# polimi-ispl/deep_prior_interpolation

Hardware: AMD Instinct MI355X
Metric: Adam iters/sec on 3D MultiRes-UNet (whole job over n_gpus; per_gpu beside it); recon SNR(dB) vs ref under config.snr_vs_reference (higher is better)
Workload: dtype f32

## Files before the change

### deep_prior_interpolation_amd/_lib.py

```python
import ctypes as C
import os

_HERE = os.path.dirname(os.path.abspath(__file__))
LIB_PATH = os.path.join(_HERE, "libdpi_hip.so")


class DpiError(RuntimeError):
    pass


ABI_VERSION = 406

IO_X_BF16, IO_Y_BF16, IO_DY_BF16, IO_DX_BF16 = 1, 2, 4, 8
STORE_FWD_BF16, STORE_GRAD_BF16 = 1, 2


class ConvDesc(C.Structure):
    _fields_ = [("size", C.c_int), ("Cin", C.c_int), ("Cout", C.c_int), ("D", C.c_int), ("H", C.c_int), ("W", C.c_int),
                ("k", C.c_int), ("kd", C.c_int), ("stride", C.c_int), ("precision", C.c_int), ("io", C.c_int)]

    def __init__(self, Cin=0, Cout=0, D=1, H=1, W=1, k=1, kd=1, stride=1, precision=0, io=0):
        super().__init__(C.sizeof(ConvDesc), int(Cin), int(Cout), int(D), int(H), int(W), int(k), int(kd), int(stride), int(precision), int(io))


# ... 11 lines not shown

SIGNATURES = {
    "dpi_last_error": (C.c_char_p, []),
    "dpi_version": (_I, []),
    "dpi_conv_desc_size": (_I, []),
    "dpi_device_info": (_I, [_I, C.POINTER(_I), C.POINTER(_I), C.POINTER(_Z), C.c_char_p, _I]),
    "dpi_profile_marker": (_I, [_I, _P]),
    "dpi_conv_fwd_stat_blocks": (_I, [_DESC]),
    "dpi_conv_fwd": (_I, [_DESC, _P, _P, _P, _P, _P, _P, _P]),
    "dpi_conv_bwd_data": (_I, [_DESC, _P, _P, _P, _I, _P]),
    "dpi_conv_fwd_ws_floats": (_Z, [_DESC]),
    "dpi_conv_bwd_data_ws_floats": (_Z, [_DESC]),
    "dpi_conv_fwd_ws": (_I, [_DESC, _P, _P, _P, _P, _P, _P, _P, _Z, _P]),
    "dpi_conv_bwd_data_ws": (_I, [_DESC, _P, _P, _P, _I, _P, _Z, _P]),
    "dpi_conv_bwd_data_dual": (_I, [_DESC, _P, _P, _DESC, _P, _P, _P, _I, _P, _Z, _P]),
    "dpi_conv_bwd_weight_ws_floats": (_Z, [_DESC]),
    "dpi_conv_bwd_weight": (_I, [_DESC, _P, _P, _P, _P, _P, _Z, _P]),
    "dpi_stat_blocks": (_I, [_I, _Z]),
    "dpi_channel_stats": (_I, [_P, _P, _I, _Z, _P, _P]),
    "dpi_bn_finalize": (_I, [_P, _I, _I, _Z, _P, _P, _F, _F, _F, _I, _P, _P, _P, _P, _P, _P, _P]),
    "dpi_chain_apply": (_I, [_P, _P, _I, _Z, _P, _P]),
    "dpi_bn_bwd_reduce": (_I, [_P, _P, _P, _P, _P, _P, _F, _F, _I, _Z, _P, _P]),
    "dpi_bn_bwd_apply": (_I, [_P, _P, _P, _P, _P, _P, _F, _F, _P, _I, _I, _Z, _P, _P, _P, _P]),
    "dpi_bn_bwd_apply_fork": (_I, [_P, _P, _P, _P, _P, _P, _F, _F, _P, _I, _I, _Z, _P, _P, _P,
                                   _P, _P, _P, _P, _P, _F, _P, _P, _P, _P, _P, _P, _F, _P, _P]),
    "dpi_bn_bwd_apply_dual": (_I, [_P, _I, _I, _Z] + [_P, _P, _P, _P, _P, _F, _P, _P, _P, _P] * 2 + [_I, _I, _P, _P, _P, _F, _P, _P]),
    "dpi_chain_add_stats": (_I, [_P, _P, _P, _P, _I, _Z, _F, _P, _P, _P]),
    "dpi_lrelu_bwd": (_I, [_P, _P, _F, _Z, _P, _P]),
    "dpi_act_fwd": (_I, [_P, _Z, _I, _P, _P]),
    "dpi_act_bwd": (_I, [_P, _P, _Z, _I, _P, _P]),
# ... 99 lines not shown
```

### deep_prior_interpolation_amd/csrc/api.cpp

```cpp
#include <stdarg.h>
#include <string.h>
#include "common.h"

static thread_local char g_err[512] = "";

void dpi_set_error(const char* fmt, ...) {
  va_list ap;
  va_start(ap, fmt);
  vsnprintf(g_err, sizeof(g_err), fmt, ap);
  va_end(ap);
}

int dpi_check_launch(const char* what) {
  const hipError_t e = hipGetLastError();
  if (e != hipSuccess) {
    dpi_set_error("%s: %s", what, hipGetErrorString(e));
    return DPI_E_LAUNCH;
  }
  return DPI_OK;
}

extern "C" const char* dpi_last_error(void) { return g_err; }
extern "C" int dpi_version(void) { return 406; }
extern "C" int dpi_conv_desc_size(void) { return (int)sizeof(dpi_conv_desc); }
// ... 17 lines not shown

__global__ void dpi_marker_kernel() {}

extern "C" int dpi_profile_marker(int id, void* stream) {
  DPI_REQUIRE(id >= 1 && id < 65536, "profile_marker: id %d out of range", id);
  dpi_marker_kernel<<<(unsigned)id, 64, 0, (hipStream_t)stream>>>();
  return dpi_check_launch("profile_marker");
}

extern "C" int dpi_set_option(const char* key, int value) {
  DPI_REQUIRE(key != nullptr, "set_option: key is NULL");
  struct Entry { const char* key; int lo, hi; void (*set)(int); };
  static const Entry table[] = {
      {"splitk", 0, 1, dpi_set_splitk},
      {"dual_bwd_data", 0, 1, dpi_set_dual_bwd_data},
      {"bw_pair", 0, 2, dpi_set_bw_pair},
      {"bw_workgroups", 1, 1 << 24, [](int v) { dpi_set_bw_tuning(v, -1); }},
      {"bw_xcd_order", 0, 1, [](int v) { dpi_set_bw_tuning(0, v); }},
      {"mfma_min_cout", 0, 1 << 20, dpi_set_mfma_min_cout},
      {"bwd_weight_mfma_min_cout", 0, 1 << 20, dpi_set_bwd_weight_mfma_min_cout},
      {"fewco_mfma", 0, 1, dpi_set_fewco_mfma},
      {"q4", 0, 2, [](int v) { dpi_set_q4(v, -1); }},
      {"q4_ck", 0, 4, [](int v) { dpi_set_q4(-1, v); }},
      {"q4_debug", 0, 0xFFFF, dpi_set_q4_debug},
      {"bf16_debug", 0, 0x7F, dpi_set_bf16_debug},
  };
  for (const Entry& e : table)
    if (strcmp(key, e.key) == 0) {
      DPI_REQUIRE(value >= e.lo && value <= e.hi && !(strcmp(key, "q4_ck") == 0 && value != 0 && value != 2 && value != 4),
                  "set_option: %s = %d out of range [%d, %d]", key, value, e.lo, e.hi);
// ... 7 lines not shown
```

### deep_prior_interpolation_amd/csrc/conv_direct.hip

```cpp
#include "conv_kernels.h"

namespace {

struct ConvArgs {
  const float* __restrict__ x;
  const float* __restrict__ chain;
  const float* __restrict__ w;
  const float* __restrict__ bias;
  float* __restrict__ y;
  double* __restrict__ partials;
  int Cin, Cout;
  int D, H, W;
  int Do, Ho, Wo;
  int ntd, nth, ntw;
  long w_out_stride, w_in_stride;
  int accumulate;
  int xb, yb;
};

template <int KD, int S, int CO_B, int OW, int TZ, int TY, int TX, int CI_B, bool FLIP>
__global__ __launch_bounds__(TZ* TY* TX) void conv_direct_kernel(ConvArgs a) {
  constexpr int KS = 3;
  constexpr int NT = TZ * TY * TX;
  constexpr int SD = (KD > 1) ? S : 1;
// ... 485 lines not shown
}

extern "C" int dpi_conv_fwd_ws(const dpi_conv_desc* d, const float* x, const float* x_chain, const float* w, const float* bias, float* y,
                               double* stat_partials, float* ws, size_t ws_floats, void* stream) {
  if (int e = dpi_check_conv_desc(d)) return e;
  DPI_REQUIRE(x && w && y, "conv_fwd: null tensor");
  DPI_REQUIRE(ws || ws_floats == 0, "conv_fwd: workspace size without a workspace");
  return conv_run(d, x, x_chain, w, bias, y, stat_partials, false, 0, ws, ws_floats, (hipStream_t)stream);
}

extern "C" int dpi_conv_fwd(const dpi_conv_desc* d, const float* x, const float* x_chain, const float* w,
                            const float* bias, float* y, double* stat_partials, void* stream) {
  return dpi_conv_fwd_ws(d, x, x_chain, w, bias, y, stat_partials, nullptr, 0, stream);
}

extern "C" int dpi_conv_bwd_data(const dpi_conv_desc* d, const float* dy, const float* w, float* dx,
                                 int accumulate, void* stream) {
  return dpi_conv_bwd_data_ws(d, dy, w, dx, accumulate, nullptr, 0, stream);
}

static int g_dual = getenv("DPI_NO_DUAL") ? 0 : 1;
extern "C" void dpi_set_dual_bwd_data(int on) { g_dual = on; }
extern "C" int dpi_conv_bwd_data_dual(const dpi_conv_desc* d3, const float* dy3, const float* w3, const dpi_conv_desc* d1, const float* dy1,
                                      const float* w1, float* dx, int accumulate, float* ws, size_t ws_floats, void* stream) {
  if (int e = dpi_check_conv_desc(d3)) return e;
  if (int e = dpi_check_conv_desc(d1)) return e;
  DPI_REQUIRE(dy3 && w3 && dy1 && w1 && dx, "conv_bwd_data_dual: null tensor");
  DPI_REQUIRE(ws || ws_floats == 0, "conv_bwd_data_dual: workspace size without a workspace");
  DPI_REQUIRE(d3->k == 3 && d1->k == 1 && d3->stride == 1 && d1->stride == 1, "conv_bwd_data_dual: needs a 3x3(x3) and a 1x1(x1) stride-1 layer");
  DPI_REQUIRE(d3->Cin == d1->Cin && d3->D == d1->D && d3->H == d1->H && d3->W == d1->W, "conv_bwd_data_dual: the two layers read different tensors");
// ... 33 lines not shown
```

### deep_prior_interpolation_amd/csrc/conv_kernels.h

```cpp
#pragma once
#include "common.h"

struct MfmaSecond { const float* x2; const float* w2; int C2; long w2_co_stride, w2_c_stride; };
void dpi_conv_out_dims(const dpi_conv_desc* d, int* Do, int* Ho, int* Wo);
int dpi_conv_mfma_stat_blocks(const dpi_conv_desc* d, bool flip);
size_t dpi_conv_mfma_ws_floats(const dpi_conv_desc* d, bool flip);
bool dpi_conv_mfma_second_ok(const dpi_conv_desc* d, bool flip, int C2, bool have_ws);
int dpi_conv_mfma_run(const dpi_conv_desc* d, const float* x, const float* chain, const float* w, const float* bias, float* y,
                      double* partials, bool flip, int accumulate, float* ws, size_t ws_floats, hipStream_t st, const MfmaSecond* sec = nullptr);
int dpi_conv_bwd_data_s2_mfma_run(const dpi_conv_desc* d, const float* dy, const float* w, float* dx, int accumulate, hipStream_t st);
size_t dpi_conv_bwd_weight_mfma_ws_floats(const dpi_conv_desc* d);
bool dpi_conv_bwd_weight_mfma_swapped(const dpi_conv_desc* d, bool chained);
int dpi_conv_bwd_weight_mfma_run(const dpi_conv_desc* d, const float* x, const float* chain, const float* dy, float* dw, float* ws, hipStream_t st);
size_t dpi_conv_bwd_weight_smallco_ws_floats(const dpi_conv_desc* d);
int dpi_conv_bwd_weight_smallco_run(const dpi_conv_desc* d, const float* x, const float* chain, const float* dy, float* dw, float* ws, hipStream_t st);
int dpi_conv_pw_mfma_stat_blocks(const dpi_conv_desc* d);
int dpi_conv_pw_mfma_run(const dpi_conv_desc* d, const float* x, const float* chain, const float* w, const float* bias, float* y,
                         double* partials, bool flip, int accumulate, hipStream_t st);
size_t dpi_conv_pw_bwd_weight_mfma_ws_floats(const dpi_conv_desc* d);
int dpi_conv_pw_bwd_weight_mfma_run(const dpi_conv_desc* d, const float* x, const float* chain, const float* dy, float* dw, float* ws, hipStream_t st);
bool dpi_conv_fewco_usable(const dpi_conv_desc* d);
int dpi_conv_fewco_stat_blocks(const dpi_conv_desc* d);
int dpi_conv_fewco_mfma_run(const dpi_conv_desc* d, const float* x, const float* chain, const float* w, const float* bias, float* y,
                            double* partials, hipStream_t st);
bool dpi_conv_q4_usable(const dpi_conv_desc* d, bool flip);
int dpi_conv_q4_stat_blocks(const dpi_conv_desc* d);
int dpi_conv_q4_run(const dpi_conv_desc* d, const float* x, const float* chain, const float* w, const float* bias, float* y,
                    double* partials, bool flip, int accumulate, hipStream_t st);
bool dpi_bf16_force_all();
bool dpi_conv_bf16_usable(const dpi_conv_desc* d, bool flip);
int dpi_conv_bf16_stat_blocks(const dpi_conv_desc* d);
bool dpi_conv_bf16_second_ok(const dpi_conv_desc* d, bool flip);
int dpi_conv_bf16_run(const dpi_conv_desc* d, const float* x, const float* chain, const float* w, const float* bias, float* y,
                      double* partials, bool flip, int accumulate, hipStream_t st, const MfmaSecond* sec = nullptr);
bool dpi_conv_bf16_s2_usable(const dpi_conv_desc* d);
int dpi_conv_bf16_s2_stat_blocks(const dpi_conv_desc* d);
int dpi_conv_bf16_s2_run(const dpi_conv_desc* d, const float* x, const float* chain, const float* w, const float* bias, float* y, double* partials,
                         hipStream_t st);
bool dpi_conv_bf16_s2_bwd_usable(const dpi_conv_desc* d);
int dpi_conv_bf16_s2_bwd_run(const dpi_conv_desc* d, const float* dy, const float* w, float* dx, int accumulate, hipStream_t st);
bool dpi_conv_bf16_bww_usable(const dpi_conv_desc* d);
size_t dpi_conv_bf16_bww_ws_floats(const dpi_conv_desc* d);
int dpi_conv_bf16_bww_run(const dpi_conv_desc* d, const float* x, const float* chain, const float* dy, float* dw, float* ws, hipStream_t st);
// ... 4 lines not shown
```

### deep_prior_interpolation_amd/csrc/conv_q4_mfma.hip

```cpp
#include "conv_kernels.h"

namespace {

typedef float f32x4 __attribute__((ext_vector_type(4)));

struct QArgs {
  const float* __restrict__ x;
  const float* __restrict__ chain;
  const float* __restrict__ w;
  const float* __restrict__ bias;
  float* __restrict__ y;
  double* __restrict__ partials;
  int Cin, Cout;
  int D, H, W;
  int ntd, nth, ntw;
  long w_out_stride, w_in_stride;
  int accumulate;
  int dbg;
};

template <int R>
struct QGeo {
  static constexpr int TZ = 4, TY = R, TW = 64;
  static constexpr int ID = TZ + 2, IH = R + 2;
  static constexpr int RS = 72;
  static constexpr int DS = IH * RS, CS = ID * DS;
  static constexpr int NV4 = ID * IH * 18;
  static constexpr int E = (NV4 + 255) / 256;
};

__device__ __forceinline__ int q4_xcd_tile(int bid, int ntiles) {
  const int q = ntiles >> 3, r = ntiles & 7, xcd = bid & 7, i = bid >> 3;
  return (xcd < r ? xcd * (q + 1) : r * (q + 1) + (xcd - r) * q) + i;
// ... 202 lines not shown

template <int R>
struct QiGeo {
  static constexpr int TZ = 4, TY = R, TW = 64;
  static constexpr int ID = TZ + 2, IH = R + 2;
  static constexpr int NP = 72;
  static constexpr int RS = NP * 4, DS = IH * RS, TILE = ID * DS;
  static constexpr int NSLOT = ID * IH * 18;
  static constexpr int E = (NSLOT + 255) / 256;
};
__device__ __forceinline__ int qi_pos(int col) {
  const int g = col >> 2, j = col & 3;
  return (4 * g + (j ^ ((g >> 1) & 3))) * 4;
}

template <int R, int NB, bool FLIP, bool AL, bool KHP = false>
__global__ __launch_bounds__(256, 2) void conv_q4i_mfma_kernel(QArgs a) {
  static_assert(!KHP || (NB == 1 && !FLIP), "kh-packed rows: one output channel, forward only");
  using G = QiGeo<R>;
  constexpr int TAPS = 27;
  constexpr int NWT = KHP ? 9 * 16 : TAPS * NB * 16;
  constexpr int WE = (NWT + 255) / 256;
  __shared__ __attribute__((aligned(16))) float lds[G::TILE];
  __shared__ __attribute__((aligned(16))) float wl[NWT];
  __shared__ double red[4][4 * NB][2];

  const int tid = threadIdx.x, lane = tid & 63, wid = tid >> 6;
  const int ntiles = a.ntd * a.nth * a.ntw;
  const int tile_id = q4_xcd_tile(blockIdx.x, ntiles);
  int bt = tile_id;
  const int tw_i = bt % a.ntw; bt /= a.ntw;
  const int th_i = bt % a.nth; bt /= a.nth;
  const int od0 = bt * G::TZ, oh0 = th_i * G::TY, ow0 = tw_i * G::TW;
  const size_t V = (size_t)a.D * a.H * a.W;

  int goff[G::E], loff[G::E];
#pragma unroll
  for (int e = 0; e < G::E; ++e) {
    const int idx = tid + e * 256;
    const int q = idx % 18, row = idx / 18;
    const int hy = row % G::IH, dz = row / G::IH;
    const int gd = od0 - 1 + dz, gh = oh0 - 1 + hy, gw = ow0 - 4 + 4 * q;
    const bool ok = idx < G::NSLOT && gd >= 0 && gd < a.D && gh >= 0 && gh < a.H && gw >= 0 && gw + 4 <= a.W;
    goff[e] = ok ? (gd * a.H + gh) * a.W + gw : -4;
    loff[e] = idx < G::NSLOT ? dz * G::DS + hy * G::RS + 16 * q : -1;
  }
  const int swz = ((tid % 18) >> 1) & 3;
  auto stage_load = [&](f32x4 (&sr)[G::E][4], int c0) {
#pragma unroll
    for (int c = 0; c < 4; ++c) {
      const int ci = min(c0 + c, a.Cin - 1);
      const __amdgpu_buffer_rsrc_t r = dpi_buffer(a.x + (size_t)ci * V, V * sizeof(float));
#pragma unroll
      for (int e = 0; e < G::E; ++e) {
        if constexpr (AL) sr[e][c] = __builtin_bit_cast(f32x4, __builtin_amdgcn_raw_buffer_load_b128(r, goff[e] * 4, 0, 0));
        else {
#pragma unroll
          for (int k = 0; k < 4; ++k) sr[e][c][k] = dpi_buffer_load(r, goff[e] < 0 ? -4 : (goff[e] + k) * 4);
        }
// ... 44 lines not shown
  auto load_wt = [&](float (&wreg)[WE], int c0) {
#pragma unroll
    for (int k = 0; k < WE; ++k) {
      bool ok;
      wreg[k] = a.w[wt_index(tid + k * 256, c0, ok)];
    }
  };
  auto store_wt = [&](const float (&wreg)[WE], int c0) {
#pragma unroll
    for (int k = 0; k < WE; ++k) {
      bool ok;
      wt_index(tid + k * 256, c0, ok);
      if (tid + k * 256 < NWT) wl[tid + k * 256] = ok ? wreg[k] : 0.f;
    }
  };

  const int Do = a.D, Ho = a.H, Wo = a.W;
  const int od = od0 + wid, ow = ow0 + lane;
  f32x4 acc[R][NB];
#pragma unroll
  for (int hr = 0; hr < R; ++hr)
#pragma unroll
    for (int s = 0; s < NB; ++s) acc[hr][s] = (f32x4){0.f, 0.f, 0.f, 0.f};
  f32x4 accp[KHP ? G::IH : 1][2];
#pragma unroll
  for (int q = 0; q < (KHP ? G::IH : 1); ++q) { accp[q][0] = (f32x4){0.f, 0.f, 0.f, 0.f}; accp[q][1] = (f32x4){0.f, 0.f, 0.f, 0.f}; }

  f32x4 sr[G::E][4];
  float wreg[WE];
  load_wt(wreg, 0);
  stage_load(sr, 0);

  int xoff[3];
#pragma unroll
  for (int kw = 0; kw < 3; ++kw) xoff[kw] = wid * G::DS + qi_pos(3 + lane + kw);
  const f32x4* __restrict__ wl4 = reinterpret_cast<const f32x4*>(wl) + (lane & 3);

  for (int c0 = 0; c0 < a.Cin; c0 += 4) {
    __syncthreads();
    if (!(a.dbg & 2) || c0 == 0) stage_store(sr, c0);
    store_wt(wreg, c0);
    __syncthreads();
    auto load_x = [&](f32x4 (&xv)[3], int kd, int ir) {
#pragma unroll
      for (int kw = 0; kw < 3; ++kw) xv[kw] = *reinterpret_cast<const f32x4*>(lds + xoff[kw] + kd * G::DS + ir * G::RS);
    };
    auto load_w = [&](f32x4 (&wr)[9][NB], int kd) {
      if constexpr (KHP) {
#pragma unroll
        for (int kw = 0; kw < 3; ++kw) wr[kw][0] = wl4[(kd * 3 + kw) * 4];
      } else {
#pragma unroll
        for (int t = 0; t < 9; ++t)
#pragma unroll
          for (int s = 0; s < NB; ++s) wr[t][s] = wl4[((kd * 9 + t) * NB + s) * 4];
      }
    };
    f32x4 wr[9][NB], xv[3], xn[3];
    load_w(wr, 0);
    load_x(xv, 0, 0);
    __builtin_amdgcn_sched_barrier(0);
    if (c0 + 4 < a.Cin) {
      load_wt(wreg, c0 + 4);
      if (!(a.dbg & 1)) stage_load(sr, c0 + 4);
    }
    __builtin_amdgcn_sched_barrier(0);
#pragma unroll
    for (int kd = 0; kd < 3; ++kd) {
#pragma unroll
      for (int ir = 0; ir < G::IH; ++ir) {
        if (ir + 1 < G::IH) load_x(xn, kd, ir + 1);
        else if (kd + 1 < 3) load_x(xn, kd + 1, 0);
        __builtin_amdgcn_sched_barrier(0);
        if constexpr (KHP) {
#pragma unroll
          for (int kw = 0; kw < 3; ++kw)
#pragma unroll
            for (int c = 0; c < 4; ++c)
              accp[ir][c & 1] = __builtin_amdgcn_mfma_f32_4x4x1f32(wr[kw][0][c], xv[kw][c], accp[ir][c & 1], 0, 0, 0);
        } else {
#pragma unroll
        for (int kw = 0; kw < 3; ++kw)
#pragma unroll
          for (int c = 0; c < 4; ++c)
#pragma unroll
            for (int kh = 0; kh < 3; ++kh) {
              const int hr = ir - kh;
              if (hr >= 0 && hr < R) {
#pragma unroll
                for (int s = 0; s < NB; ++s)
                  acc[hr][s] = __builtin_amdgcn_mfma_f32_4x4x1f32(wr[kh * 3 + kw][s][c], xv[kw][c], acc[hr][s], 0, 0, 0);
              }
            }
        }
        __builtin_amdgcn_sched_barrier(0);
#pragma unroll
        for (int kw = 0; kw < 3; ++kw) xv[kw] = xn[kw];
      }
      if (kd + 1 < 3) load_w(wr, kd + 1);
    }
  }

  if constexpr (KHP) {
#pragma unroll
    for (int hr = 0; hr < R; ++hr)
      acc[hr][0][0] = ((accp[hr][0][0] + accp[hr][1][0]) + (accp[hr + 1][0][1] + accp[hr + 1][1][1])) + (accp[hr + 2][0][2] + accp[hr + 2][1][2]);
  }
  const bool col_ok = od < Do && ow < Wo;
#pragma unroll
  for (int s = 0; s < NB; ++s)
#pragma unroll
    for (int i = 0; i < 4; ++i) {
      const int co = 4 * s + i;
      const bool cok = co < a.Cout;
      const float bv = (a.bias && cok) ? a.bias[co] : 0.f;
      float* __restrict__ yc = a.y + (size_t)(cok ? co : 0) * V + ((size_t)(od < Do ? od : 0) * Ho + oh0) * Wo + ow;
      double sm = 0.0, sq = 0.0;
      float old[R];
      if (a.accumulate) {
#pragma unroll
        for (int hr = 0; hr < R; ++hr) old[hr] = (cok && col_ok && oh0 + hr < Ho) ? yc[hr * Wo] : 0.f;
      } else {
#pragma unroll
        for (int hr = 0; hr < R; ++hr) old[hr] = 0.f;
      }
#pragma unroll
      for (int hr = 0; hr < R; ++hr) {
        if (cok && col_ok && oh0 + hr < Ho) {
          const float v = acc[hr][s][i] + bv + old[hr];
          if (!(a.dbg & 8)) yc[hr * Wo] = v;
          sm += v;
          sq += (double)v * v;
        }
      }
      if (a.partials && cok) {
        sm = wave_sum(sm);
        sq = wave_sum(sq);
        if (lane == 0) { red[wid][co][0] = sm; red[wid][co][1] = sq; }
      }
    }
  if (a.partials) {
    __syncthreads();
    if (tid < 2 * a.Cout) {
      const int c = tid >> 1, which = tid & 1;
      a.partials[((size_t)tile_id * a.Cout + c) * 2 + which] = red[0][c][which] + red[1][c][which] + red[2][c][which] + red[3][c][which];
    }
  }
}

static int g_q4 = 1;
static int g_q4_ck = 0;
static int g_q4_dbg = 0;
static int g_q4_khp = getenv("DPI_NO_KHP") ? 0 : 1;

}

extern "C" void dpi_set_q4_debug(int flags) { g_q4_dbg = flags; }
extern "C" void dpi_set_q4(int on, int ck) {
  if (on >= 0) g_q4 = on;
  if (ck == 0 || ck == 2 || ck == 4) g_q4_ck = ck;
// ... 36 lines not shown
  if (aligned) conv_q4_mfma_kernel<8, NB, 2, FLIP, true><<<ntiles, 256, extra, st>>>(a);
  else conv_q4_mfma_kernel<8, NB, 2, FLIP, false><<<ntiles, 256, extra, st>>>(a);
}

int dpi_conv_q4_run(const dpi_conv_desc* d, const float* x, const float* chain, const float* w, const float* bias, float* y,
                    double* partials, bool flip, int accumulate, hipStream_t st) {
  const int cin = flip ? d->Cout : d->Cin, cout = flip ? d->Cin : d->Cout;
  const long w_out = flip ? 27 : (long)d->Cin * 27, w_in = flip ? (long)d->Cin * 27 : 27;
  QArgs a{x, chain, w, bias, y, partials, cin, cout, d->D, d->H, d->W, 0, 0, 0, w_out, w_in, accumulate, g_q4_dbg};
  const int ntiles = q4_tiles(d, &a.ntd, &a.nth, &a.ntw);
  const bool aligned = ((uintptr_t)x & 15) == 0;
  if (cout <= 4) { if (flip) q4_launch<1, true>(a, ntiles, aligned, st); else q4_launch<1, false>(a, ntiles, aligned, st); }
  else { if (flip) q4_launch<2, true>(a, ntiles, aligned, st); else q4_launch<2, false>(a, ntiles, aligned, st); }
  return dpi_check_launch("conv_q4_mfma");
}
```

### deep_prior_interpolation_amd/csrc/dpi_hip_internal.h

```cpp
#pragma once
#define DPI_INTERNAL __attribute__((visibility("hidden")))
extern "C" {
DPI_INTERNAL void dpi_set_bw_tuning(int want_workgroups, int xcd_order);
DPI_INTERNAL void dpi_set_bf16_debug(int flags);
DPI_INTERNAL void dpi_set_splitk(int on);
DPI_INTERNAL void dpi_set_dual_bwd_data(int on);
DPI_INTERNAL void dpi_set_bw_pair(int mode);
DPI_INTERNAL void dpi_set_mfma_min_cout(int n);
DPI_INTERNAL void dpi_set_bwd_weight_mfma_min_cout(int n);
DPI_INTERNAL void dpi_set_fewco_mfma(int on);
DPI_INTERNAL void dpi_set_q4(int on, int ck);
DPI_INTERNAL void dpi_set_q4_debug(int flags);
}
```

### deep_prior_interpolation_amd/ops.py

```python
import ctypes as C
import os
import threading

import torch

from . import _lib
from ._lib import ConvDesc, check, ptr, stream

BN_EPS = 1e-5
BN_MOMENTUM = 0.1


def _req(t, name, act=False):
    if not t.is_cuda:
        raise _lib.DpiError("%s must live on the GPU: the HIP path has no CPU fallback" % name)
    if t.dtype != torch.float32 and not (act and t.dtype == torch.bfloat16):
        raise _lib.DpiError("%s must be float32%s (got %s)" % (name, " or bfloat16" if act else "", t.dtype))
    return t.contiguous()


STORAGE_BF16 = os.environ.get("DPI_STORAGE", "fp32") == "bf16"
_tls = threading.local()


# ... 162 lines not shown
_ws_cache = {}


def _ws_floats(kind, d):
    key = (kind, d.Cin, d.Cout, d.D, d.H, d.W, d.k, d.kd, d.stride, d.precision, d.io)
    n = _ws_cache.get(key)
    if n is None:
        L = _lib.load()
        n = {"fwd": L.dpi_conv_fwd_ws_floats, "bwd_data": L.dpi_conv_bwd_data_ws_floats}[kind](C.byref(d))
        _ws_cache[key] = n
    return n


def reset_ws_cache():
    _ws_cache.clear()


def _conv_ws(n, like):
    return torch.empty(n, dtype=torch.float32, device=like.device) if n else None


def raw_conv_fwd(d, x, chain, w, bias, y, partials=None):
    L = _lib.load()
    n = _ws_floats("fwd", d)
    ws = _conv_ws(n, x)
    _timed("conv_fwd", d, lambda: check(L.dpi_conv_fwd_ws(C.byref(d), ptr(x), ptr(chain), ptr(w), ptr(bias), ptr(y),
                                                          ptr(partials), ptr(ws), n, stream()), "dpi_conv_fwd"))


def raw_conv_bwd_data(d, dy, w, dx, accumulate=False):
    L = _lib.load()
    n = _ws_floats("bwd_data", d)
    ws = _conv_ws(n, dy)
    _timed("conv_bwd_data", d, lambda: check(L.dpi_conv_bwd_data_ws(C.byref(d), ptr(dy), ptr(w), ptr(dx), int(accumulate),
                                                                    ptr(ws), n, stream()), "dpi_conv_bwd_data"))


def raw_conv_bwd_data_dual(d3, dy3, w3, d1, dy1, w1, dx, accumulate=False):
    L = _lib.load()
    n = _ws_floats("bwd_data", d3)
    ws = _conv_ws(n, dy3)

# ... 471 lines not shown
                raw_conv_bwd_data(d, dr, w, dx)
        if ctx.has_bias and ctx.needs_input_grad[2]:
            db = _zeros_like_or_none(ctx.bias_ref, dr)
        join_weight_grads()
        return dx, dw, db, dgamma, dbeta, None, None, None, None, None, None


def _cba_raw(d, x, in_chain, w, b, bn, slope, r_out, mi_out, chain_out):
    L = _lib.load()
    nblk = L.dpi_conv_fwd_stat_blocks(C.byref(d))
    part = torch.empty(nblk * d.Cout * 2, dtype=torch.float64, device=x.device)
    raw_conv_fwd(d, x, in_chain, w, b, r_out, part)
    Do, Ho, Wo = desc_out_dims(d)
    raw_bn_finalize(part, nblk, d.Cout, Do * Ho * Wo, bn.weight, bn.bias, slope, bn.running_mean, bn.running_var,
                    bn.num_batches_tracked, mi_out, chain_out)


DEAD_BIAS = "off"


def _zeros_like_or_none(b, dr=None):
    if b is None or DEAD_BIAS == "off":
        return None
    if DEAD_BIAS == "noise":
        return torch.randn_like(b) * 1e-6
    return dr.sum(dim=[0] + list(range(2, dr.ndim)), dtype=torch.float32)


class Block3dFn(torch.autograd.Function):

# ... 16 lines not shown
        r1, r2, r3 = R[:, :c1], R[:, c1:c1 + c2], R[:, c1 + c2:]
        ch1, ch2, ch3 = CH[:c1 * 5], CH[c1 * 5:(c1 + c2) * 5], CH[(c1 + c2) * 5:]
        mi1, mi2, mi3 = (torch.empty(2 * c, **f32) for c in (c1, c2, c3))
        miA, miS, miB = (torch.empty(2 * Ct, **f32) for _ in range(3))
        dsc = make_desc(x, ws, 1, adt)
        S = torch.empty_like(R)
        chSA = torch.empty((2, Ct * 5), **f32)
        chS, chA = chSA[0], chSA[1]
        side_shortcut = BRANCH_SHORTCUT if branch_on() else 0

        def shortcut_on_branch():
            with _Branch("short", x, S, miS, chS):
                _cba_raw(dsc, x, None, ws, bs, bns_, slope, S, miS, chS)
        if side_shortcut == 1:
            shortcut_on_branch()
        _cba_raw(d1, x, None, w1, b1, bn1_, slope, r1, mi1, ch1)
        if side_shortcut == 2:
            shortcut_on_branch()
        d2 = make_desc(r1, w2, 1, adt)
        _cba_raw(d2, r1, ch1, w2, b2, bn2_, slope, r2, mi2, ch2)
        d3 = make_desc(r2, w3, 1, adt)
        _cba_raw(d3, r2, ch2, w3, b3, bn3_, slope, r3, mi3, ch3)
        A = blk.bn1
        raw_bn_stats_finalize(R, CH, Ct, V, gA, eA, 1.0, A.running_mean, A.running_var, A.num_batches_tracked, miA, chA,
                              compose=True)
        if side_shortcut:
            join_branch("short")
        else:
            _cba_raw(dsc, x, None, ws, bs, bns_, slope, S, miS, chS)
        y = torch.empty_like(R)
        tless = _join_fused_ok(R, S)
        t = _join_forward(S, chS, R, chA, Ct, V, slope, blk.bn2, gB, eB, miB, y, keep_t=not tless)
        if tless:
            t = chSA
        ctx.tless = tless
        ctx.save_for_backward(x, R, S, t, CH, mi1, mi2, mi3, miA, miS, miB, *[q for q in p if q is not None])
        ctx.none_mask = [q is None for q in p]
        ctx.descs = (d1, d2, d3, dsc)
        ctx.slope = float(slope)
        ctx.split = (c1, c2, c3)
        return y

    @staticmethod
# ... 63 lines not shown
        x = _req(x, "respath input", act=True)
        (w3, b3, g3, e3, w1, b1, g1, e1, gB, eB) = p
        L = _lib.load()
        f32 = dict(dtype=torch.float32, device=x.device)
        adt = act_dtype()
        Ct = w3.shape[0]
        bn3_, bn1_ = rp.conv3x3._parts()[1], rp.conv1x1._parts()[1]
        d3, d1 = make_desc(x, w3, 1, adt), make_desc(x, w1, 1, adt)
        Do, Ho, Wo = desc_out_dims(d3)
        V = Do * Ho * Wo
        r3 = torch.empty(_like_spatial(x, Ct, Do, Ho, Wo), dtype=adt, device=x.device)
        r1 = torch.empty_like(r3)
        mi3, mi1, miB = (torch.empty(2 * Ct, **f32) for _ in range(3))
        ch13 = torch.empty((2, 5 * Ct), **f32)
        ch1, ch3 = ch13[0], ch13[1]
        _cba_raw(d3, x, None, w3, b3, bn3_, slope, r3, mi3, ch3)
        _cba_raw(d1, x, None, w1, b1, bn1_, slope, r1, mi1, ch1)
        y = torch.empty_like(r3)
        tless = _join_fused_ok(r3, r1)
        t = _join_forward(r1, ch1, r3, ch3, Ct, V, slope, rp.bn, gB, eB, miB, y, keep_t=not tless)
        if tless:
            t = ch13
        ctx.tless = tless
        ctx.save_for_backward(x, r3, r1, t, mi3, mi1, miB, *[q for q in p if q is not None])
        ctx.none_mask = [q is None for q in p]
        ctx.descs = (d3, d1)
        ctx.slope = float(slope)
        return y

    @staticmethod
    def backward(ctx, dy):
        dy = _req(dy, "respath grad", act=True)
# ... 33 lines not shown
    T["cat"] = torch.empty(_like_spatial(x, Cs + Cd, Do, Ho, Wo), dtype=adt, device=x.device)
    return T


def _skip_tensors(T):
    return [T[k] for k in ("r3", "r1", "t", "mi3", "mi1", "miB", "ch13", "chB", "cat")]


def _skip_launch(x, rp, slope, p, T):
    (w3, b3, g3, e3, w1, b1, g1, e1, gB, eB) = p
    L = _lib.load()
    Cs = T["Cs"]
    Do, Ho, Wo = T["dims"]
    V = Do * Ho * Wo
    bn3_, bn1_ = rp.conv3x3._parts()[1], rp.conv1x1._parts()[1]
    _cba_raw(T["d3"], x, None, w3, b3, bn3_, slope, T["r3"], T["mi3"], T["ch3"])
    _cba_raw(T["d1"], x, None, w1, b1, bn1_, slope, T["r1"], T["mi1"], T["ch1"])
    nblk = L.dpi_stat_blocks(Cs, V)
    part = torch.empty(nblk * Cs * 2, dtype=torch.float64, device=x.device)
    tless = T["tless"]
    check(L.dpi_chain_add_stats_io(ptr(T["r1"]), ptr(T["ch1"]), ptr(T["r3"]), ptr(T["ch3"]), Cs, V, slope, None if tless else ptr(T["t"]),
                                   ptr(part), _io(T["r3"]), stream()), "dpi_chain_add_stats")
    B = rp.bn
    raw_bn_finalize(part, nblk, Cs, V, gB, eB, slope, B.running_mean, B.running_var, B.num_batches_tracked, T["miB"], T["chB"],
                    act_first=1)
    if tless:
        check(L.dpi_chain_add_apply(ptr(T["r1"]), ptr(T["ch1"]), ptr(T["r3"]), ptr(T["ch3"]), ptr(T["chB"]), Cs, V, ptr(T["cat"][:, :Cs]),
                                    _io(T["r3"]), stream()), "dpi_chain_add_apply")
    else:
        raw_chain_apply(T["t"], T["chB"], Cs, V, T["cat"][:, :Cs])


# ... 433 lines not shown
```

### include/dpi_hip.h

```cpp
#ifndef DPI_HIP_H
#define DPI_HIP_H

#include <stddef.h>
#include <stdint.h>

#ifdef __cplusplus
extern "C" {
#endif

#define DPI_OK 0
#define DPI_E_ARG (-1)
#define DPI_E_LAUNCH (-2)
#define DPI_E_WORKSPACE (-3)

#define DPI_CHAIN_STRIDE 5

const char* dpi_last_error(void);
int dpi_version(void);
int dpi_device_info(int device, int* cus, int* lds_bytes, size_t* hbm_bytes, char* name, int name_len);
int dpi_profile_marker(int id, void* stream);
int dpi_set_option(const char* key, int value);

typedef struct {
  int size;
// ... 12 lines not shown

int dpi_conv_fwd_stat_blocks(const dpi_conv_desc* d);
int dpi_conv_fwd(const dpi_conv_desc* d, const float* x, const float* x_chain, const float* w,
                 const float* bias, float* y, double* stat_partials, void* stream);
int dpi_conv_bwd_data(const dpi_conv_desc* d, const float* dy, const float* w, float* dx,
                      int accumulate, void* stream);
size_t dpi_conv_fwd_ws_floats(const dpi_conv_desc* d);
size_t dpi_conv_bwd_data_ws_floats(const dpi_conv_desc* d);
int dpi_conv_fwd_ws(const dpi_conv_desc* d, const float* x, const float* x_chain, const float* w,
                    const float* bias, float* y, double* stat_partials, float* ws, size_t ws_floats, void* stream);
int dpi_conv_bwd_data_ws(const dpi_conv_desc* d, const float* dy, const float* w, float* dx,
                         int accumulate, float* ws, size_t ws_floats, void* stream);
int dpi_conv_bwd_data_dual(const dpi_conv_desc* d3, const float* dy3, const float* w3,
                           const dpi_conv_desc* d1, const float* dy1, const float* w1,
                           float* dx, int accumulate, float* ws, size_t ws_floats, void* stream);
size_t dpi_conv_bwd_weight_ws_floats(const dpi_conv_desc* d);
int dpi_conv_bwd_weight(const dpi_conv_desc* d, const float* x, const float* x_chain, const float* dy,
                        float* dw, float* ws, size_t ws_floats, void* stream);


int dpi_stat_blocks(int C, size_t V);
int dpi_channel_stats(const float* x, const float* chain, int C, size_t V, double* partials, void* stream);
int dpi_bn_finalize(const double* partials, int nblk, int C, size_t count, const float* gamma,
                    const float* beta, float eps, float momentum, float slope, int act_first,
                    const float* in_chain, float* running_mean, float* running_var, int64_t* num_batches_tracked,
                    float* mean_invstd, float* chain_out, void* stream);
int dpi_chain_apply(const float* x, const float* chain, int C, size_t V, float* y, void* stream);
int dpi_bn_bwd_reduce(const float* dy, const float* x, const float* mean_invstd, const float* gamma,
                      const float* beta, const float* in_chain, float pre_slope, float post_slope, int C,
                      size_t V, double* partials, void* stream);
// ... 151 lines not shown
```

Before: 32.77.

## Fuse sibling 1x1 conv into Q4 MFMA 3x3 forward kernel sharing input tiles

```diff
diff --git a/deep_prior_interpolation_amd/_lib.py b/deep_prior_interpolation_amd/_lib.py
--- a/deep_prior_interpolation_amd/_lib.py
+++ b/deep_prior_interpolation_amd/_lib.py
@@ -49,6 +49,8 @@
     "dpi_conv_fwd_ws": (_I, [_DESC, _P, _P, _P, _P, _P, _P, _P, _Z, _P]),
     "dpi_conv_bwd_data_ws": (_I, [_DESC, _P, _P, _P, _I, _P, _Z, _P]),
     "dpi_conv_bwd_data_dual": (_I, [_DESC, _P, _P, _DESC, _P, _P, _P, _I, _P, _Z, _P]),
+    "dpi_conv_fwd_dual_ok": (_I, [_DESC, _I]),
+    "dpi_conv_fwd_dual": (_I, [_DESC, _P, _P, _P, _P, _P, _P, _P, _P, _P, _P, _I, _P]),
     "dpi_conv_bwd_weight_ws_floats": (_Z, [_DESC]),
     "dpi_conv_bwd_weight": (_I, [_DESC, _P, _P, _P, _P, _P, _Z, _P]),
     "dpi_stat_blocks": (_I, [_I, _Z]),
diff --git a/deep_prior_interpolation_amd/csrc/api.cpp b/deep_prior_interpolation_amd/csrc/api.cpp
--- a/deep_prior_interpolation_amd/csrc/api.cpp
+++ b/deep_prior_interpolation_amd/csrc/api.cpp
@@ -55,6 +55,7 @@
   static const Entry table[] = {
       {"splitk", 0, 1, dpi_set_splitk},
       {"dual_bwd_data", 0, 1, dpi_set_dual_bwd_data},
+      {"dual_fwd", 0, 1, dpi_set_dual_fwd},
       {"bw_pair", 0, 2, dpi_set_bw_pair},
       {"bw_workgroups", 1, 1 << 24, [](int v) { dpi_set_bw_tuning(v, -1); }},
       {"bw_xcd_order", 0, 1, [](int v) { dpi_set_bw_tuning(0, v); }},
diff --git a/deep_prior_interpolation_amd/csrc/conv_direct.hip b/deep_prior_interpolation_amd/csrc/conv_direct.hip
--- a/deep_prior_interpolation_amd/csrc/conv_direct.hip
+++ b/deep_prior_interpolation_amd/csrc/conv_direct.hip
@@ -523,6 +523,24 @@
   return dpi_conv_fwd_ws(d, x, x_chain, w, bias, y, stat_partials, nullptr, 0, stream);
 }
 
+static int g_fwd_dual = getenv("DPI_NO_FWD_DUAL") ? 0 : 1;
+extern "C" void dpi_set_dual_fwd(int on) { g_fwd_dual = on; }
+static bool fwd_dual_plan(const dpi_conv_desc* d, int Cout2) {
+  if (!g_fwd_dual || d->k != 3 || d->kd != 3 || d->stride != 1 || d->precision != 0 || d->io != 0) return false;
+  return conv_plan(d, false, 0).kernel == ConvKernel::Q4 && dpi_conv_q4_dual_ok(d, Cout2);
+}
+extern "C" int dpi_conv_fwd_dual_ok(const dpi_conv_desc* d, int Cout2) {
+  return dpi_check_conv_desc(d) == DPI_OK && fwd_dual_plan(d, Cout2) ? 1 : 0;
+}
+extern "C" int dpi_conv_fwd_dual(const dpi_conv_desc* d, const float* x, const float* x_chain, const float* w, const float* bias, float* y,
+                                 double* stat_partials, const float* w2, const float* bias2, float* y2, double* stat_partials2, int Cout2,
+                                 void* stream) {
+  if (int e = dpi_check_conv_desc(d)) return e;
+  DPI_REQUIRE(x && w && y && w2 && y2, "conv_fwd_dual: null tensor");
+  DPI_REQUIRE(fwd_dual_plan(d, Cout2), "conv_fwd_dual: no fused launch for this pair (ask dpi_conv_fwd_dual_ok; run dpi_conv_fwd twice)");
+  return dpi_conv_q4_dual_run(d, x, x_chain, w, bias, y, stat_partials, w2, bias2, y2, stat_partials2, Cout2, (hipStream_t)stream);
+}
+
 extern "C" int dpi_conv_bwd_data(const dpi_conv_desc* d, const float* dy, const float* w, float* dx,
                                  int accumulate, void* stream) {
   return dpi_conv_bwd_data_ws(d, dy, w, dx, accumulate, nullptr, 0, stream);
diff --git a/deep_prior_interpolation_amd/csrc/conv_kernels.h b/deep_prior_interpolation_amd/csrc/conv_kernels.h
--- a/deep_prior_interpolation_amd/csrc/conv_kernels.h
+++ b/deep_prior_interpolation_amd/csrc/conv_kernels.h
@@ -27,6 +27,9 @@
 int dpi_conv_q4_stat_blocks(const dpi_conv_desc* d);
 int dpi_conv_q4_run(const dpi_conv_desc* d, const float* x, const float* chain, const float* w, const float* bias, float* y,
                     double* partials, bool flip, int accumulate, hipStream_t st);
+bool dpi_conv_q4_dual_ok(const dpi_conv_desc* d, int Cout2);
+int dpi_conv_q4_dual_run(const dpi_conv_desc* d, const float* x, const float* chain, const float* w, const float* bias, float* y,
+                         double* partials, const float* w2, const float* bias2, float* y2, double* partials2, int Cout2, hipStream_t st);
 bool dpi_bf16_force_all();
 bool dpi_conv_bf16_usable(const dpi_conv_desc* d, bool flip);
 int dpi_conv_bf16_stat_blocks(const dpi_conv_desc* d);
diff --git a/deep_prior_interpolation_amd/csrc/conv_q4_mfma.hip b/deep_prior_interpolation_amd/csrc/conv_q4_mfma.hip
--- a/deep_prior_interpolation_amd/csrc/conv_q4_mfma.hip
+++ b/deep_prior_interpolation_amd/csrc/conv_q4_mfma.hip
@@ -17,6 +17,11 @@
   long w_out_stride, w_in_stride;
   int accumulate;
   int dbg;
+  const float* __restrict__ w2;
+  const float* __restrict__ bias2;
+  float* __restrict__ y2;
+  double* __restrict__ partials2;
+  int Cout2;
 };
 
 template <int R>
@@ -249,9 +254,56 @@
   return (4 * g + (j ^ ((g >> 1) & 3))) * 4;
 }
 
-template <int R, int NB, bool FLIP, bool AL, bool KHP = false>
+template <int R, int NBX>
+__device__ __forceinline__ void q4i_epilogue(const f32x4 (&acc)[R][NBX], int Cout, const float* __restrict__ bias, float* __restrict__ y,
+                                             bool stats, double (*red)[2], bool first, size_t V, int od, int oh0, int ow, int Do, int Ho, int Wo,
+                                             int lane, int accumulate, int dbg) {
+  const bool col_ok = od < Do && ow < Wo;
+#pragma unroll
+  for (int s = 0; s < NBX; ++s)
+#pragma unroll
+    for (int i = 0; i < 4; ++i) {
+      const int co = 4 * s + i;
+      const bool cok = co < Cout;
+      const float bv = (bias && cok) ? bias[co] : 0.f;
+      float* __restrict__ yc = y + (size_t)(cok ? co : 0) * V + ((size_t)(od < Do ? od : 0) * Ho + oh0) * Wo + ow;
+      double sm = 0.0, sq = 0.0;
+      float old[R];
+      if (accumulate) {
+#pragma unroll
+        for (int hr = 0; hr < R; ++hr) old[hr] = (cok && col_ok && oh0 + hr < Ho) ? yc[hr * Wo] : 0.f;
+      } else {
+#pragma unroll
+        for (int hr = 0; hr < R; ++hr) old[hr] = 0.f;
+      }
+#pragma unroll
+      for (int hr = 0; hr < R; ++hr) {
+        if (cok && col_ok && oh0 + hr < Ho) {
+          const float v = acc[hr][s][i] + bv + old[hr];
+          if (!(dbg & 8)) yc[hr * Wo] = v;
+          sm += v;
+          sq += (double)v * v;
+        }
+      }
+      if (stats && cok) {
+        sm = wave_sum(sm);
+        sq = wave_sum(sq);
+        if (lane == 0) {
+          if (first) { red[co][0] = sm; red[co][1] = sq; }
+          else { red[co][0] += sm; red[co][1] += sq; }
+        }
+      }
+    }
+}
+
+template <int R, int NB, bool FLIP, bool AL, bool KHP = false, int NB2 = 0, int NS = 1>
 __global__ __launch_bounds__(256, 2) void conv_q4i_mfma_kernel(QArgs a) {
   static_assert(!KHP || (NB == 1 && !FLIP), "kh-packed rows: one output channel, forward only");
+  static_assert(NB2 == 0 || (!FLIP && !KHP), "second output: forward only");
+  constexpr int NWT2 = NB2 * 16;
+  constexpr bool XDB = NB2 == 0;
+  __shared__ __attribute__((aligned(16))) float wl2[NWT2 ? NWT2 : 4];
+  __shared__ double red2[4][NB2 ? 4 * NB2 : 1][2];
   using G = QiGeo<R>;
   constexpr int TAPS = 27;
   constexpr int NWT = KHP ? 9 * 16 : TAPS * NB * 16;
@@ -266,18 +318,27 @@
   int bt = tile_id;
   const int tw_i = bt % a.ntw; bt /= a.ntw;
   const int th_i = bt % a.nth; bt /= a.nth;
-  const int od0 = bt * G::TZ, oh0 = th_i * G::TY, ow0 = tw_i * G::TW;
+  const int od0 = bt * G::TZ, oh0 = th_i * (G::TY * NS), ow0 = tw_i * G::TW;
   const size_t V = (size_t)a.D * a.H * a.W;
 
   int goff[G::E], loff[G::E];
+  auto set_goff = [&](int oh) {
+#pragma unroll
+    for (int e = 0; e < G::E; ++e) {
+      const int idx = tid + e * 256;
+      const int q = idx % 18, row = idx / 18;
+      const int hy = row % G::IH, dz = row / G::IH;
+      const int gd = od0 - 1 + dz, gh = oh - 1 + hy, gw = ow0 - 4 + 4 * q;
+      const bool ok = idx < G::NSLOT && gd >= 0 && gd < a.D && gh >= 0 && gh < a.H && gw >= 0 && gw + 4 <= a.W;
+      goff[e] = ok ? (gd * a.H + gh) * a.W + gw : -4;
+    }
+  };
+  set_goff(oh0);
 #pragma unroll
   for (int e = 0; e < G::E; ++e) {
     const int idx = tid + e * 256;
     const int q = idx % 18, row = idx / 18;
     const int hy = row % G::IH, dz = row / G::IH;
-    const int gd = od0 - 1 + dz, gh = oh0 - 1 + hy, gw = ow0 - 4 + 4 * q;
-    const bool ok = idx < G::NSLOT && gd >= 0 && gd < a.D && gh >= 0 && gh < a.H && gw >= 0 && gw + 4 <= a.W;
-    goff[e] = ok ? (gd * a.H + gh) * a.W + gw : -4;
     loff[e] = idx < G::NSLOT ? dz * G::DS + hy * G::RS + 16 * q : -1;
   }
   const int swz = ((tid % 18) >> 1) & 3;
@@ -352,32 +413,56 @@
       if (tid + k * 256 < NWT) wl[tid + k * 256] = ok ? wreg[k] : 0.f;
     }
   };
+  auto wt2_index = [&](int c0, bool& ok) {
+    const int c = tid & 3, co2 = tid >> 2, ci = c0 + c;
+    ok = tid < NWT2 && co2 < a.Cout2 && ci < a.Cin;
+    return (ok ? co2 : 0) * a.Cin + (ok ? ci : 0);
+  };
+  auto load_wt2 = [&](float& w2reg, int c0) {
+    if constexpr (NB2 > 0) { bool ok; w2reg = a.w2[wt2_index(c0, ok)]; }
+  };
+  auto store_wt2 = [&](float w2reg, int c0) {
+    if constexpr (NB2 > 0) { bool ok; wt2_index(c0, ok); if (tid < NWT2) wl2[tid] = ok ? w2reg : 0.f; }
+  };
 
   const int Do = a.D, Ho = a.H, Wo = a.W;
   const int od = od0 + wid, ow = ow0 + lane;
-  f32x4 acc[R][NB];
-#pragma unroll
-  for (int hr = 0; hr < R; ++hr)
-#pragma unroll
-    for (int s = 0; s < NB; ++s) acc[hr][s] = (f32x4){0.f, 0.f, 0.f, 0.f};
-  f32x4 accp[KHP ? G::IH : 1][2];
-#pragma unroll
-  for (int q = 0; q < (KHP ? G::IH : 1); ++q) { accp[q][0] = (f32x4){0.f, 0.f, 0.f, 0.f}; accp[q][1] = (f32x4){0.f, 0.f, 0.f, 0.f}; }
 
   f32x4 sr[G::E][4];
-  float wreg[WE];
+  float wreg[WE], w2reg = 0.f;
   load_wt(wreg, 0);
+  load_wt2(w2reg, 0);
   stage_load(sr, 0);
 
   int xoff[3];
 #pragma unroll
   for (int kw = 0; kw < 3; ++kw) xoff[kw] = wid * G::DS + qi_pos(3 + lane + kw);
   const f32x4* __restrict__ wl4 = reinterpret_cast<const f32x4*>(wl) + (lane & 3);
+  const f32x4* __restrict__ wl24 = reinterpret_cast<const f32x4*>(wl2) + (lane & 3);
+
+#pragma unroll 1
+  for (int sub = 0; sub < NS; ++sub) {
+  const int oh0s = oh0 + sub * R;
+  if (NS > 1 && sub > 0 && oh0s >= Ho) break;
+  f32x4 acc[R][NB];
+#pragma unroll
+  for (int hr = 0; hr < R; ++hr)
+#pragma unroll
+    for (int s = 0; s < NB; ++s) acc[hr][s] = (f32x4){0.f, 0.f, 0.f, 0.f};
+  f32x4 acc2[R][NB2 ? NB2 : 1];
+#pragma unroll
+  for (int hr = 0; hr < R; ++hr)
+#pragma unroll
+    for (int s = 0; s < (NB2 ? NB2 : 1); ++s) acc2[hr][s] = (f32x4){0.f, 0.f, 0.f, 0.f};
+  f32x4 accp[KHP ? G::IH : 1][2];
+#pragma unroll
+  for (int q = 0; q < (KHP ? G::IH : 1); ++q) { accp[q][0] = (f32x4){0.f, 0.f, 0.f, 0.f}; accp[q][1] = (f32x4){0.f, 0.f, 0.f, 0.f}; }
 
   for (int c0 = 0; c0 < a.Cin; c0 += 4) {
     __syncthreads();
     if (!(a.dbg & 2) || c0 == 0) stage_store(sr, c0);
     store_wt(wreg, c0);
+    store_wt2(w2reg, c0);
     __syncthreads();
     auto load_x = [&](f32x4 (&xv)[3], int kd, int ir) {
 #pragma unroll
@@ -400,15 +485,25 @@
     __builtin_amdgcn_sched_barrier(0);
     if (c0 + 4 < a.Cin) {
       load_wt(wreg, c0 + 4);
+      load_wt2(w2reg, c0 + 4);
       if (!(a.dbg & 1)) stage_load(sr, c0 + 4);
+    } else if constexpr (NS > 1) {
+      if (sub + 1 < NS && oh0s + R < Ho) {
+        set_goff(oh0s + R);
+        load_wt(wreg, 0);
+        load_wt2(w2reg, 0);
+        stage_load(sr, 0);
+      }
     }
     __builtin_amdgcn_sched_barrier(0);
 #pragma unroll
     for (int kd = 0; kd < 3; ++kd) {
 #pragma unroll
       for (int ir = 0; ir < G::IH; ++ir) {
-        if (ir + 1 < G::IH) load_x(xn, kd, ir + 1);
-        else if (kd + 1 < 3) load_x(xn, kd + 1, 0);
+        if constexpr (XDB) {
+          if (ir + 1 < G::IH) load_x(xn, kd, ir + 1);
+          else if (kd + 1 < 3) load_x(xn, kd + 1, 0);
+        }
         __builtin_amdgcn_sched_barrier(0);
         if constexpr (KHP) {
 #pragma unroll
@@ -430,10 +525,28 @@
                   acc[hr][s] = __builtin_amdgcn_mfma_f32_4x4x1f32(wr[kh * 3 + kw][s][c], xv[kw][c], acc[hr][s], 0, 0, 0);
               }
             }
+          if constexpr (NB2 > 0) {
+            if (kd == 1 && ir >= 1 && ir <= R) {
+#pragma unroll
+              for (int s = 0; s < NB2; s += 2) {
+                const f32x4 wa = wl24[s * 4], wb = wl24[(s + 1 < NB2 ? s + 1 : s) * 4];
+#pragma unroll
+                for (int c = 0; c < 4; ++c) {
+                  acc2[ir - 1][s] = __builtin_amdgcn_mfma_f32_4x4x1f32(wa[c], xv[1][c], acc2[ir - 1][s], 0, 0, 0);
+                  if (s + 1 < NB2) acc2[ir - 1][s + 1] = __builtin_amdgcn_mfma_f32_4x4x1f32(wb[c], xv[1][c], acc2[ir - 1][s + 1], 0, 0, 0);
+                }
+              }
+            }
+          }
         }
         __builtin_amdgcn_sched_barrier(0);
-#pragma unroll
-        for (int kw = 0; kw < 3; ++kw) xv[kw] = xn[kw];
+        if constexpr (XDB) {
+#pragma unroll
+          for (int kw = 0; kw < 3; ++kw) xv[kw] = xn[kw];
+        } else {
+          if (ir + 1 < G::IH) load_x(xv, kd, ir + 1);
+          else if (kd + 1 < 3) load_x(xv, kd + 1, 0);
+        }
       }
       if (kd + 1 < 3) load_w(wr, kd + 1);
     }
@@ -444,44 +557,21 @@
     for (int hr = 0; hr < R; ++hr)
       acc[hr][0][0] = ((accp[hr][0][0] + accp[hr][1][0]) + (accp[hr + 1][0][1] + accp[hr + 1][1][1])) + (accp[hr + 2][0][2] + accp[hr + 2][1][2]);
   }
-  const bool col_ok = od < Do && ow < Wo;
-#pragma unroll
-  for (int s = 0; s < NB; ++s)
-#pragma unroll
-    for (int i = 0; i < 4; ++i) {
-      const int co = 4 * s + i;
-      const bool cok = co < a.Cout;
-      const float bv = (a.bias && cok) ? a.bias[co] : 0.f;
-      float* __restrict__ yc = a.y + (size_t)(cok ? co : 0) * V + ((size_t)(od < Do ? od : 0) * Ho + oh0) * Wo + ow;
-      double sm = 0.0, sq = 0.0;
-      float old[R];
-      if (a.accumulate) {
-#pragma unroll
-        for (int hr = 0; hr < R; ++hr) old[hr] = (cok && col_ok && oh0 + hr < Ho) ? yc[hr * Wo] : 0.f;
-      } else {
-#pragma unroll
-        for (int hr = 0; hr < R; ++hr) old[hr] = 0.f;
-      }
-#pragma unroll
-      for (int hr = 0; hr < R; ++hr) {
-        if (cok && col_ok && oh0 + hr < Ho) {
-          const float v = acc[hr][s][i] + bv + old[hr];
-          if (!(a.dbg & 8)) yc[hr * Wo] = v;
-          sm += v;
-          sq += (double)v * v;
-        }
-      }
-      if (a.partials && cok) {
-        sm = wave_sum(sm);
-        sq = wave_sum(sq);
-        if (lane == 0) { red[wid][co][0] = sm; red[wid][co][1] = sq; }
-      }
-    }
-  if (a.partials) {
+  q4i_epilogue<R, NB>(acc, a.Cout, a.bias, a.y, a.partials != nullptr, red[wid], sub == 0, V, od, oh0s, ow, Do, Ho, Wo, lane, a.accumulate, a.dbg);
+  if constexpr (NB2 > 0)
+    q4i_epilogue<R, NB2>(acc2, a.Cout2, a.bias2, a.y2, a.partials2 != nullptr, red2[wid], sub == 0, V, od, oh0s, ow, Do, Ho, Wo, lane, 0, a.dbg);
+  }
+  if (a.partials || (NB2 > 0 && a.partials2)) {
     __syncthreads();
-    if (tid < 2 * a.Cout) {
+    if (a.partials && tid < 2 * a.Cout) {
       const int c = tid >> 1, which = tid & 1;
       a.partials[((size_t)tile_id * a.Cout + c) * 2 + which] = red[0][c][which] + red[1][c][which] + red[2][c][which] + red[3][c][which];
+    }
+    if constexpr (NB2 > 0) {
+      if (a.partials2 && tid < 2 * a.Cout2) {
+        const int c = tid >> 1, which = tid & 1;
+        a.partials2[((size_t)tile_id * a.Cout2 + c) * 2 + which] = red2[0][c][which] + red2[1][c][which] + red2[2][c][which] + red2[3][c][which];
+      }
     }
   }
 }
@@ -548,3 +638,25 @@
   else { if (flip) q4_launch<2, true>(a, ntiles, aligned, st); else q4_launch<2, false>(a, ntiles, aligned, st); }
   return dpi_check_launch("conv_q4_mfma");
 }
+
+static const int g_q4_dual_pays = getenv("DPI_Q4_DUAL") ? atoi(getenv("DPI_Q4_DUAL")) : 0;
+bool dpi_conv_q4_dual_ok(const dpi_conv_desc* d, int Cout2) {
+  if (!dpi_conv_q4_usable(d, false) || Cout2 < 1 || Cout2 > 28) return false;
+  return g_q4 == 2 || (g_q4_dual_pays && d->Cout <= 4);
+}
+
+int dpi_conv_q4_dual_run(const dpi_conv_desc* d, const float* x, const float* chain, const float* w, const float* bias, float* y,
+                         double* partials, const float* w2, const float* bias2, float* y2, double* partials2, int Cout2, hipStream_t st) {
+  QArgs a{x, chain, w, bias, y, partials, d->Cin, d->Cout, d->D, d->H, d->W, 0, 0, 0, (long)d->Cin * 27, 27, 0, g_q4_dbg & 0xff,
+          w2, bias2, y2, partials2, Cout2};
+  const int ntiles = q4_tiles(d, &a.ntd, &a.nth, &a.ntw);
+  const bool aligned = ((uintptr_t)x & 15) == 0;
+  if (d->Cout <= 4) {
+    if (aligned) conv_q4i_mfma_kernel<4, 1, false, true, false, 7, 2><<<ntiles, 256, 0, st>>>(a);
+    else conv_q4i_mfma_kernel<4, 1, false, false, false, 7, 2><<<ntiles, 256, 0, st>>>(a);
+  } else {
+    if (aligned) conv_q4i_mfma_kernel<2, 2, false, true, false, 7, 4><<<ntiles, 256, 0, st>>>(a);
+    else conv_q4i_mfma_kernel<2, 2, false, false, false, 7, 4><<<ntiles, 256, 0, st>>>(a);
+  }
+  return dpi_check_launch("conv_q4_mfma (dual)");
+}
diff --git a/deep_prior_interpolation_amd/csrc/dpi_hip_internal.h b/deep_prior_interpolation_amd/csrc/dpi_hip_internal.h
--- a/deep_prior_interpolation_amd/csrc/dpi_hip_internal.h
+++ b/deep_prior_interpolation_amd/csrc/dpi_hip_internal.h
@@ -5,6 +5,7 @@
 DPI_INTERNAL void dpi_set_bf16_debug(int flags);
 DPI_INTERNAL void dpi_set_splitk(int on);
 DPI_INTERNAL void dpi_set_dual_bwd_data(int on);
+DPI_INTERNAL void dpi_set_dual_fwd(int on);
 DPI_INTERNAL void dpi_set_bw_pair(int mode);
 DPI_INTERNAL void dpi_set_mfma_min_cout(int n);
 DPI_INTERNAL void dpi_set_bwd_weight_mfma_min_cout(int n);
diff --git a/deep_prior_interpolation_amd/ops.py b/deep_prior_interpolation_amd/ops.py
--- a/deep_prior_interpolation_amd/ops.py
+++ b/deep_prior_interpolation_amd/ops.py
@@ -200,6 +200,7 @@
 
 def reset_ws_cache():
     _ws_cache.clear()
+    _dual_ok_cache.clear()
 
 
 def _conv_ws(n, like):
@@ -212,6 +213,26 @@
     ws = _conv_ws(n, x)
     _timed("conv_fwd", d, lambda: check(L.dpi_conv_fwd_ws(C.byref(d), ptr(x), ptr(chain), ptr(w), ptr(bias), ptr(y),
                                                           ptr(partials), ptr(ws), n, stream()), "dpi_conv_fwd"))
+
+
+FWD_DUAL = os.environ.get("DPI_FWD_DUAL", "1") == "1"
+_dual_ok_cache = {}
+
+
+def conv_fwd_dual_ok(d3, d1):
+    if not FWD_DUAL or d1.k != 1 or (d1.Cin, d1.D, d1.H, d1.W, d1.stride, d1.precision, d1.io) != (d3.Cin, d3.D, d3.H, d3.W, 1, d3.precision, d3.io):
+        return False
+    key = (d3.Cin, d3.Cout, d3.D, d3.H, d3.W, d3.k, d3.kd, d3.stride, d3.precision, d3.io, d1.Cout)
+    ok = _dual_ok_cache.get(key)
+    if ok is None:
+        ok = _dual_ok_cache[key] = bool(_lib.load().dpi_conv_fwd_dual_ok(C.byref(d3), d1.Cout))
+    return ok
+
+
+def raw_conv_fwd_dual(d3, x, chain, w3, b3, y3, part3, w1, b1, y1, part1):
+    L = _lib.load()
+    _timed("conv_fwd", d3, lambda: check(L.dpi_conv_fwd_dual(C.byref(d3), ptr(x), ptr(chain), ptr(w3), ptr(b3), ptr(y3), ptr(part3),
+                                                             ptr(w1), ptr(b1), ptr(y1), ptr(part1), int(w1.shape[0]), stream()), "dpi_conv_fwd_dual"))
 
 
 def raw_conv_bwd_data(d, dy, w, dx, accumulate=False):
@@ -713,6 +734,18 @@
     Do, Ho, Wo = desc_out_dims(d)
     raw_bn_finalize(part, nblk, d.Cout, Do * Ho * Wo, bn.weight, bn.bias, slope, bn.running_mean, bn.running_var,
                     bn.num_batches_tracked, mi_out, chain_out)
+
+
+def _cba_raw_dual(d3, d1, x, in_chain, w3, b3, bn3, r3, mi3, ch3, w1, b1, bn1, r1, mi1, ch1, slope):
+    L = _lib.load()
+    nblk = L.dpi_conv_fwd_stat_blocks(C.byref(d3))
+    part3 = torch.empty(nblk * d3.Cout * 2, dtype=torch.float64, device=x.device)
+    part1 = torch.empty(nblk * d1.Cout * 2, dtype=torch.float64, device=x.device)
+    raw_conv_fwd_dual(d3, x, in_chain, w3, b3, r3, part3, w1, b1, r1, part1)
+    Do, Ho, Wo = desc_out_dims(d3)
+    for part, d, bn, mi, ch in ((part3, d3, bn3, mi3, ch3), (part1, d1, bn1, mi1, ch1)):
+        raw_bn_finalize(part, nblk, d.Cout, Do * Ho * Wo, bn.weight, bn.bias, slope, bn.running_mean, bn.running_var,
+                        bn.num_batches_tracked, mi, ch)
 
 
 DEAD_BIAS = "off"
@@ -759,7 +792,11 @@
                 _cba_raw(dsc, x, None, ws, bs, bns_, slope, S, miS, chS)
         if side_shortcut == 1:
             shortcut_on_branch()
-        _cba_raw(d1, x, None, w1, b1, bn1_, slope, r1, mi1, ch1)
+        fused_shortcut = not BRANCH_SHORTCUT and conv_fwd_dual_ok(d1, dsc)
+        if fused_shortcut:
+            _cba_raw_dual(d1, dsc, x, None, w1, b1, bn1_, r1, mi1, ch1, ws, bs, bns_, S, miS, chS, slope)
+        else:
+            _cba_raw(d1, x, None, w1, b1, bn1_, slope, r1, mi1, ch1)
         if side_shortcut == 2:
             shortcut_on_branch()
         d2 = make_desc(r1, w2, 1, adt)
@@ -771,7 +808,7 @@
                               compose=True)
         if side_shortcut:
             join_branch("short")
-        else:
+        elif not fused_shortcut:
             _cba_raw(dsc, x, None, ws, bs, bns_, slope, S, miS, chS)
         y = torch.empty_like(R)
         tless = _join_fused_ok(R, S)
@@ -865,8 +902,11 @@
         mi3, mi1, miB = (torch.empty(2 * Ct, **f32) for _ in range(3))
         ch13 = torch.empty((2, 5 * Ct), **f32)
         ch1, ch3 = ch13[0], ch13[1]
-        _cba_raw(d3, x, None, w3, b3, bn3_, slope, r3, mi3, ch3)
-        _cba_raw(d1, x, None, w1, b1, bn1_, slope, r1, mi1, ch1)
+        if conv_fwd_dual_ok(d3, d1):
+            _cba_raw_dual(d3, d1, x, None, w3, b3, bn3_, r3, mi3, ch3, w1, b1, bn1_, r1, mi1, ch1, slope)
+        else:
+            _cba_raw(d3, x, None, w3, b3, bn3_, slope, r3, mi3, ch3)
+            _cba_raw(d1, x, None, w1, b1, bn1_, slope, r1, mi1, ch1)
         y = torch.empty_like(r3)
         tless = _join_fused_ok(r3, r1)
         t = _join_forward(r1, ch1, r3, ch3, Ct, V, slope, rp.bn, gB, eB, miB, y, keep_t=not tless)
@@ -930,8 +970,11 @@
     Do, Ho, Wo = T["dims"]
     V = Do * Ho * Wo
     bn3_, bn1_ = rp.conv3x3._parts()[1], rp.conv1x1._parts()[1]
-    _cba_raw(T["d3"], x, None, w3, b3, bn3_, slope, T["r3"], T["mi3"], T["ch3"])
-    _cba_raw(T["d1"], x, None, w1, b1, bn1_, slope, T["r1"], T["mi1"], T["ch1"])
+    if conv_fwd_dual_ok(T["d3"], T["d1"]):
+        _cba_raw_dual(T["d3"], T["d1"], x, None, w3, b3, bn3_, T["r3"], T["mi3"], T["ch3"], w1, b1, bn1_, T["r1"], T["mi1"], T["ch1"], slope)
+    else:
+        _cba_raw(T["d3"], x, None, w3, b3, bn3_, slope, T["r3"], T["mi3"], T["ch3"])
+        _cba_raw(T["d1"], x, None, w1, b1, bn1_, slope, T["r1"], T["mi1"], T["ch1"])
     nblk = L.dpi_stat_blocks(Cs, V)
     part = torch.empty(nblk * Cs * 2, dtype=torch.float64, device=x.device)
     tless = T["tless"]
diff --git a/include/dpi_hip.h b/include/dpi_hip.h
--- a/include/dpi_hip.h
+++ b/include/dpi_hip.h
@@ -50,6 +50,9 @@
 int dpi_conv_bwd_data_dual(const dpi_conv_desc* d3, const float* dy3, const float* w3,
                            const dpi_conv_desc* d1, const float* dy1, const float* w1,
                            float* dx, int accumulate, float* ws, size_t ws_floats, void* stream);
+int dpi_conv_fwd_dual_ok(const dpi_conv_desc* d, int Cout2);
+int dpi_conv_fwd_dual(const dpi_conv_desc* d, const float* x, const float* x_chain, const float* w, const float* bias, float* y,
+                      double* stat_partials, const float* w2, const float* bias2, float* y2, double* stat_partials2, int Cout2, void* stream);
 size_t dpi_conv_bwd_weight_ws_floats(const dpi_conv_desc* d);
 int dpi_conv_bwd_weight(const dpi_conv_desc* d, const float* x, const float* x_chain, const float* dy,
                         float* dw, float* ws, size_t ws_floats, void* stream);
```

Result: slower. 32.44 (-1.0%).
